# ruolin/strawberry

Measured on AMD Instinct MI355X. Metric: loci/s, EM-to-convergence (+ FPKM/TPM epilogue), C3, higher is better.
Workload: dtype f64; 1 GPU; C3 human-scale synthetic: 60000 loci/GPU, niso~1+Geom(0.25), nrow~LogNormal(ln30,1), 2e8 fragments; loci_per_gpu=60000, fragments_per_gpu=200000086, collective=none (one rank), steps_pipelined=True

## Files before the change

### include/sbgpu.h

```cpp
#ifndef SBGPU_H_
#define SBGPU_H_

#include <stdint.h>

#ifdef __cplusplus
extern "C" {
#endif

#define SBGPU_VERSION_MAJOR 0
#define SBGPU_VERSION_MINOR 1

#define SBGPU_OK 0
#define SBGPU_EINVAL (-1)
#define SBGPU_EHIP (-2)
#define SBGPU_ENODEV (-3)
#define SBGPU_ENOMEM (-4)
#define SBGPU_ESHAPE (-5)
#define SBGPU_EUNSUPPORTED (-6)
#define SBGPU_ERCCL (-7)

#define SBGPU_EM_OK 0
#define SBGPU_EM_INIT_EMPTY 1
#define SBGPU_EM_DENOM_ZERO 2
#define SBGPU_EM_MAXITER 3
// ... 11 lines not shown
   const int64_t *row_off;
   const int64_t *iso_off;
   const int64_t *f_off;
   const int32_t *count;
   const double *F;
} sbgpu_batch_t;

typedef struct {
   int32_t total_mapped_reads;
   int32_t effective_len_norm;
   int32_t filter_by_expression;
   int32_t reserved;
   double insert_mean;
   double min_isoform_frac;
} sbgpu_abundance_params_t;

const char *sbgpu_version(void);
const char *sbgpu_last_error(void);
const char *sbgpu_build_id(void);
int sbgpu_device_count(void);

int sbgpu_init(int device, sbgpu_ctx_t **ctx_out);
int sbgpu_finalize(sbgpu_ctx_t *ctx);
int64_t sbgpu_release_idle_memory(void);
int sbgpu_device_info(sbgpu_ctx_t *ctx, int64_t out[8]);
int sbgpu_synchronize(sbgpu_ctx_t *ctx, void *stream);

int sbgpu_plan_create(sbgpu_ctx_t *ctx, int64_t n_loci, const int64_t *row_off,
                      const int64_t *iso_off, const int64_t *f_off,
                      sbgpu_plan_t **plan_out);
int sbgpu_plan_destroy(sbgpu_plan_t *plan);
int sbgpu_plan_info(const sbgpu_plan_t *plan, int64_t out[8]);
int sbgpu_plan_classes(const sbgpu_plan_t *plan, int64_t *out, int cap);

int sbgpu_plan_locus_kinds(const sbgpu_plan_t *plan, int8_t *out);

int sbgpu_em_run_device(sbgpu_ctx_t *ctx, const sbgpu_plan_t *plan,
                        const int32_t *d_count, const double *d_F,
                        double *d_theta, int32_t *d_status, int32_t *d_iters,
                        void *stream);

int sbgpu_em_run_device_split(sbgpu_ctx_t *ctx, const sbgpu_plan_t *plan, const int32_t *d_count, const double *d_F,
                              double *d_theta, int32_t *d_status, int32_t *d_iters, void *fork_stream,
                              void *join_stream);

int sbgpu_em_run_device_f32(sbgpu_ctx_t *ctx, const sbgpu_plan_t *plan,
                            const int32_t *d_count, const float *d_F,
                            float *d_theta, int32_t *d_status, int32_t *d_iters,
                            void *stream);

int sbgpu_em_run_device_bias(sbgpu_ctx_t *ctx, const sbgpu_plan_t *plan, const int32_t *d_count, const double *d_F,
                             const double *d_row_bias, const double *d_iso_bias, double *d_theta, int32_t *d_status,
                             int32_t *d_iters, void *stream);
int sbgpu_em_run_device_bias_f32(sbgpu_ctx_t *ctx, const sbgpu_plan_t *plan, const int32_t *d_count, const float *d_F,
                                 const float *d_row_bias, const float *d_iso_bias, float *d_theta, int32_t *d_status,
                                 int32_t *d_iters, void *stream);

int sbgpu_set_timing(sbgpu_ctx_t *ctx, int on);
int sbgpu_last_stage_ms(sbgpu_ctx_t *ctx, int cap, float *ms, const char **names);

int sbgpu_em_last_kernel_ms(sbgpu_ctx_t *ctx, float ms[6]);

int sbgpu_em_last_phase_ms(sbgpu_ctx_t *ctx, float *ms, int cap);

int sbgpu_em_batch(sbgpu_ctx_t *ctx, const sbgpu_batch_t *host_batch,
                   double *theta_out, int32_t *status_out, int32_t *iters_out);
// ... 406 lines not shown
```

### strawberry_amd/_lib.py

```python
import ctypes as C
import os

HERE = os.path.dirname(os.path.abspath(__file__))
LIB_PATH = os.environ.get("SBGPU_LIB") or os.path.join(HERE, "lib", "libsbgpu.so")

SBGPU_OK = 0
SBGPU_EINVAL = -1
SBGPU_ESHAPE = -5
SBGPU_EUNSUPPORTED = -6
SBGPU_ERCCL = -7
EM_UNSOLVED = -1
EM_OK, EM_INIT_EMPTY, EM_DENOM_ZERO, EM_MAXITER = 0, 1, 2, 3
STATUS_NAMES = {0: "OK", 1: "INIT_EMPTY", 2: "DENOM_ZERO", 3: "MAXITER"}

SYMBOLS = [
    "sbgpu_version", "sbgpu_build_id", "sbgpu_last_error", "sbgpu_device_count", "sbgpu_init", "sbgpu_finalize",
    "sbgpu_device_info", "sbgpu_synchronize", "sbgpu_plan_create", "sbgpu_plan_destroy", "sbgpu_plan_info",
    "sbgpu_plan_classes", "sbgpu_plan_locus_kinds", "sbgpu_em_run_device", "sbgpu_em_run_device_f32", "sbgpu_em_run_device_bias", "sbgpu_em_run_device_bias_f32", "sbgpu_em_last_kernel_ms",
    "sbgpu_set_timing", "sbgpu_em_last_phase_ms", "sbgpu_last_stage_ms", "sbgpu_pair_mates_host", "sbgpu_pair_mates_device", "sbgpu_matepairs_destroy", "sbgpu_matepairs_info",
    "sbgpu_matepairs_pairs", "sbgpu_matepairs_export", "sbgpu_assign_reads_host", "sbgpu_assign_reads_device",
    "sbgpu_bam_index_host", "sbgpu_bam_decode_host", "sbgpu_bam_decode_device", "sbgpu_bamreads_destroy", "sbgpu_bamreads_info",
    "sbgpu_bamreads_reads", "sbgpu_bamreads_export",
    "sbgpu_comm_unique_id", "sbgpu_comm_init", "sbgpu_comm_info", "sbgpu_comm_rccl_ranks", "sbgpu_comm_destroy",
    "sbgpu_allreduce_sum_f64", "sbgpu_allreduce_sum_i64", "sbgpu_allreduce_sum_f64_host", "sbgpu_allreduce_sum_i64_host",
    "sbgpu_insert_pdf_table", "sbgpu_binweight_device", "sbgpu_binweight_host",
    "sbgpu_exonbin_device", "sbgpu_exonbin_host", "sbgpu_segments_host", "sbgpu_hit_features", "sbgpu_frag_lens_host",
    "sbgpu_bins_create", "sbgpu_bins_create_device", "sbgpu_bins_destroy", "sbgpu_quantify_host", "sbgpu_quantify_device",
    "sbgpu_annotation_pin", "sbgpu_annotation_unpin", "sbgpu_annotation_unpin_matching", "sbgpu_release_idle_memory",
    "sbgpu_bins_export_weights", "sbgpu_collapse_pairs_host", "sbgpu_uniq_destroy", "sbgpu_uniq_info", "sbgpu_uniq_export",
    "sbgpu_collapse_pairs_device", "sbgpu_uniq_dev_destroy", "sbgpu_uniq_dev_info", "sbgpu_uniq_dev_hits", "sbgpu_uniq_dev_export", "sbgpu_bins_info", "sbgpu_bins_grouping", "sbgpu_bins_export",
    "sbgpu_format_value", "sbgpu_format_gtf_transcript", "sbgpu_format_context_row", "sbgpu_format_context_row_seq",
    "sbgpu_binseq_device", "sbgpu_binseq_host", "sbgpu_em_batch", "sbgpu_abundance_device", "sbgpu_tpm_device",
    "sbgpu_quantify_resident", "sbgpu_allreduce_max_i64", "sbgpu_allreduce_max_i64_host", "sbgpu_comm_init_host",
    "sbgpu_front_stream_begin", "sbgpu_front_stream_push", "sbgpu_front_stream_end", "sbgpu_front_stream_info", "sbgpu_front_stream_hits",
    "sbgpu_front_stream_destroy", "sbgpu_em_run_device_split",
    "sbgpu_bgzf_index_host", "sbgpu_bgzf_inflate_host", "sbgpu_bgzf_inflate_device", "sbgpu_bam_index_device", "sbgpu_bam_index_device_info", "sbgpu_front_stream_push_bgzf",
    "sbgpu_context_table_host", "sbgpu_context_table_keep", "sbgpu_context_table_device",
    "sbgpu_bootstrap_counts_host", "sbgpu_bootstrap_counts_device", "sbgpu_em_bootstrap_device",
    "sbgpu_replicate_stats_host", "sbgpu_replicate_stats_device", "sbgpu_bootstrap_keep", "sbgpu_abundance_bootstrap_device",
    "sbgpu_locus_abundance_host", "sbgpu_locus_abundance_device", "sbgpu_locus_bootstrap_device",
    "sbgpu_fragment_assign_host", "sbgpu_fragment_assign_device",
]


class SbgpuError(RuntimeError):
    pass


class sbgpu_batch_t(C.Structure):
    _fields_ = [
        ("n_loci", C.c_int64),
        ("row_off", C.c_void_p),
        ("iso_off", C.c_void_p),
        ("f_off", C.c_void_p),
        ("count", C.c_void_p),
        ("F", C.c_void_p),
    ]


class sbgpu_abundance_params_t(C.Structure):
    _fields_ = [
        ("total_mapped_reads", C.c_int32),
        ("effective_len_norm", C.c_int32),
        ("filter_by_expression", C.c_int32),
        ("reserved", C.c_int32),
        ("insert_mean", C.c_double),
        ("min_isoform_frac", C.c_double),
    ]


class sbgpu_insert_t(C.Structure):
    _fields_ = [
        ("mean", C.c_double),
        ("sd", C.c_double),
# ... 100 lines not shown

def build():
    import subprocess
    subprocess.check_call(["make", "-s", "-C", os.path.join(HERE, "csrc")])


def load():
    global _lib
    if _lib is not None:
        return _lib
    if not os.path.exists(LIB_PATH):
        raise SbgpuError(
            "%s is missing: build it with `make -C strawberry_amd/csrc` (or __graft_entry__.build()). "
            "There is no CPU fallback." % LIB_PATH)
    try:
        import torch
    except ImportError:
        pass
    L = C.CDLL(LIB_PATH)
    vp, i64p = C.c_void_p, C.POINTER(C.c_int64)
    L.sbgpu_version.restype = C.c_char_p
    L.sbgpu_last_error.restype = C.c_char_p
    L.sbgpu_build_id.restype = C.c_char_p
    L.sbgpu_device_count.restype = C.c_int
    L.sbgpu_init.argtypes = [C.c_int, C.POINTER(vp)]
    L.sbgpu_finalize.argtypes = [vp]
    L.sbgpu_device_info.argtypes = [vp, i64p]
    L.sbgpu_synchronize.argtypes = [vp, vp]
    L.sbgpu_plan_create.argtypes = [vp, C.c_int64, vp, vp, vp, C.POINTER(vp)]
    L.sbgpu_plan_destroy.argtypes = [vp]
    L.sbgpu_plan_info.argtypes = [vp, i64p]
    L.sbgpu_plan_classes.argtypes = [vp, i64p, C.c_int]
    L.sbgpu_plan_locus_kinds.argtypes = [vp, vp]
    L.sbgpu_em_last_kernel_ms.argtypes = [vp, C.POINTER(C.c_float)]
    L.sbgpu_set_timing.argtypes = [vp, C.c_int]
    L.sbgpu_last_stage_ms.argtypes = [vp, C.c_int, C.POINTER(C.c_float), C.POINTER(C.c_char_p)]
    L.sbgpu_comm_unique_id.argtypes = [vp]
    L.sbgpu_comm_init.argtypes = [vp, C.c_int, C.c_int, vp, C.POINTER(vp)]
    L.sbgpu_comm_info.argtypes = [vp, C.POINTER(C.c_int), C.POINTER(C.c_int)]
    L.sbgpu_comm_rccl_ranks.argtypes = [vp, C.POINTER(C.c_int)]
    L.sbgpu_comm_destroy.argtypes = [vp]
    L.sbgpu_allreduce_sum_f64.argtypes = [vp, vp, C.c_int64, vp]
    L.sbgpu_allreduce_sum_i64.argtypes = [vp, vp, C.c_int64, vp]
    L.sbgpu_allreduce_sum_f64_host.argtypes = [vp, vp, C.c_int64]
    L.sbgpu_allreduce_sum_i64_host.argtypes = [vp, vp, C.c_int64]
    L.sbgpu_em_last_phase_ms.argtypes = [vp, C.POINTER(C.c_float), C.c_int]
    L.sbgpu_em_run_device.argtypes = [vp, vp, vp, vp, vp, vp, vp, vp]
    L.sbgpu_em_run_device_f32.argtypes = [vp, vp, vp, vp, vp, vp, vp, vp]
    L.sbgpu_em_run_device_split.argtypes = [vp, vp, vp, vp, vp, vp, vp, vp, vp]
    L.sbgpu_em_run_device_bias.argtypes = [vp] * 10
    L.sbgpu_em_run_device_bias_f32.argtypes = [vp] * 10
    L.sbgpu_em_batch.argtypes = [vp, C.POINTER(sbgpu_batch_t), vp, vp, vp]
    L.sbgpu_abundance_device.argtypes = [vp, vp, vp, vp, vp, C.POINTER(sbgpu_abundance_params_t), vp, vp, vp, vp, vp]
    L.sbgpu_tpm_device.argtypes = [vp, C.c_int64, vp, vp, vp, vp, vp]
    L.sbgpu_insert_pdf_table.argtypes = [C.POINTER(sbgpu_insert_t), C.c_int32, vp]
    L.sbgpu_binweight_device.argtypes = [vp, C.c_int64, vp, vp, vp, vp, vp, vp, C.c_int32, C.c_int32, C.c_int32,
                                         C.c_int32, vp, vp]
    L.sbgpu_exonbin_device.argtypes = [vp, C.POINTER(sbgpu_annotation_t), C.POINTER(sbgpu_hits_t), C.c_int32, C.c_int32,
                                       vp, vp, vp]
    L.sbgpu_exonbin_host.argtypes = [vp, C.POINTER(sbgpu_annotation_t), C.POINTER(sbgpu_hits_t), C.c_int32, C.c_int32,
                                     vp, vp]
    L.sbgpu_segments_host.argtypes = [C.c_int64, vp, vp, vp, vp, vp, vp, vp, C.c_int64]
    L.sbgpu_segments_host.restype = C.c_int64
    L.sbgpu_frag_lens_host.argtypes = [C.POINTER(sbgpu_annotation_t), C.POINTER(sbgpu_hits_t), C.c_int32, vp, vp]
    L.sbgpu_frag_lens_host.restype = C.c_int64
    L.sbgpu_hit_features.argtypes = [C.c_int, vp, vp, vp, C.c_int, vp, vp, vp, vp, vp, vp]
# ... 111 lines not shown
```

### strawberry_amd/csrc/em_device.h

```cpp
#pragma once

#include <hip/hip_runtime.h>
#include <stdint.h>

#include <type_traits>

#include "device_common.h"

namespace sb {

constexpr int kMaxIter = 1000;
constexpr double kThetaLimit = 1e-2;
constexpr double kThetaLimitSq = 0x1.a36e2eb1c432bp-14;
constexpr double kRowEps = 1e-5;

constexpr int kMaxCPLv = 8;
constexpr int32_t kStOk = 0, kStInitEmpty = 1, kStDenomZero = 2, kStMaxIter = 3;
constexpr int32_t kStRunning = 4;

template <class T>
struct EmArgsT {
   const int64_t *row_off;
   const int64_t *iso_off;
   const int64_t *f_off;
   const int32_t *count;
   const T *F;
   T *theta;
   int32_t *status;
   int32_t *iters;
   const T *row_bias = nullptr;
   const T *iso_bias = nullptr;
};
typedef EmArgsT<double> EmArgs;

struct ClassDesc {
   int32_t block_begin;
   int32_t n;
   int32_t loci_off;
   int32_t shape;
};
// ... 955 lines not shown
{
   __shared__ T s_red[NWAVES > 0 ? 2 * (kMaxCPLv + 1) * 8 * NWAVES : 1];
   set_flush_denormals<T>();
   if (NWAVES > 0) __builtin_amdgcn_s_setprio(3);
#ifdef SB_STAMPS
   const unsigned long long st0 = sb_now();
#endif
   const int n_batches = ph.total_blocks ? *ph.total_blocks : ph.n_batches;
   for (int b = (int)blockIdx.x; b < n_batches; b += (int)gridDim.x) {
   if (NWAVES > 0 && b != (int)blockIdx.x) __syncthreads();
   const int c = find_class(ph.table, ph.n_classes, b);
   const ClassDesc d = ph.table[c];
#ifdef SB_STAMPS
   if ((threadIdx.x & 63) == 0 && NWAVES == 0) {
      const unsigned wg = (blockIdx.x * (blockDim.x >> 6) + (threadIdx.x >> 6)) & (kStampWaves - 1);
      sb_debug_stamps[wg * 8 + 0] = st0;
      sb_debug_stamps[wg * 8 + 1] = sb_now();
      const unsigned hw = __builtin_amdgcn_s_getreg((31 << 11) | 4), xcc = __builtin_amdgcn_s_getreg((3 << 11) | 20);
      sb_debug_stamps[wg * 8 + 6] = ((xcc & 7u) << 10) | (((hw >> 8) & 0xFFu) << 2) | ((hw >> 4) & 3u);
   }
#endif
   ClassArgs cls;
   cls.loci = ph.lists_in + d.loci_off;
   cls.n = ph.n_in[c];
   cls.out = ph.lists_out;
   cls.out_count = ph.n_out;
   cls.route = ph.route;
   cls.next_table = ph.next_table;
   cls.it_limit = ph.it_limit;
   cls.resume = ph.resume;
   cls.batch = b - d.block_begin;
   const int layout = d.shape & 0xFF;
   const int lbG = (d.shape >> 16) & 0xFF;
#define SB_BODY(CPLV, CLV, RHALF)                                                                  \
   case (CPLV - 1) + 8 * ilog2(CLV):                                                               \
      em_tile_body<T, CPLV, CLV, tile_rows(CPLV, RHALF, RH), NWAVES>(a, cls, lbG, s_red);          \
      break;
   switch (layout) {
      SB_BODY(1, 1, 8)
      SB_BODY(2, 1, 4)
      SB_BODY(3, 1, 4)
      SB_BODY(4, 1, 4)
      SB_BODY(5, 1, 3)
      SB_BODY(6, 1, 3)
      SB_BODY(7, 1, 2)
      SB_BODY(8, 1, 2)
      SB_BODY(5, 2, 3)
      SB_BODY(6, 2, 3)
      SB_BODY(7, 2, 2)
      SB_BODY(8, 2, 2)
      SB_BODY(5, 4, 3)
      SB_BODY(6, 4, 3)
      SB_BODY(7, 4, 2)
      SB_BODY(8, 4, 2)
      SB_BODY(5, 8, 3)
      SB_BODY(6, 8, 3)
      SB_BODY(7, 8, 2)
      SB_BODY(8, 8, 2)
   default: break;
   }
#undef SB_BODY
   }
}

#ifndef SB_LAT_MAXTILE
#define SB_LAT_MAXTILE 32
#endif
constexpr int kLatMaxTile = SB_LAT_MAXTILE;
constexpr int lat_shape(int cpl, int lb_cl, int r) { return (cpl - 1) | (lb_cl << 2) | (r << 8); }
#ifndef SB_LAT_OCC
#define SB_LAT_OCC 2
#endif
#ifdef SB_COMPILE_LAT_KERNEL
__global__ __launch_bounds__(64, SB_LAT_OCC) void em_lat_kernel(EmArgs a, PhaseArgs ph)
{
   set_fp64_flush_denormals();
   const int n_batches = ph.total_blocks ? *ph.total_blocks : ph.n_batches;
   for (int b = (int)blockIdx.x; b < n_batches; b += (int)gridDim.x) {
      const int c = find_class(ph.table, ph.n_classes, b);
      const ClassDesc d = ph.table[c];
      ClassArgs cls;
      cls.loci = ph.lists_in + d.loci_off;
      cls.n = ph.n_in[c];
      cls.out = ph.lists_out;
      cls.out_count = ph.n_out;
      cls.route = ph.route;
      cls.next_table = ph.next_table;
      cls.it_limit = ph.it_limit;
      cls.resume = ph.resume;
      cls.batch = b - d.block_begin;
#define SB_LAT(CPLV, CLV, RV)                                                             \
   case lat_shape(CPLV, ilog2(CLV), RV):                                                  \
      if constexpr (CPLV * RV <= kLatMaxTile)                                             \
         em_tile_body<double, CPLV, CLV, RV, 0, true>(a, cls, 6, nullptr);                \
// ... 298 lines not shown
```

### strawberry_amd/csrc/plan.cpp

```cpp
#include "plan.h"

#include <algorithm>
#include <atomic>
#include <cstdlib>
#include <thread>
#include <map>
#include <tuple>

#include "../../include/sbgpu.h"

namespace sb {

static int64_t predicted_iterations(int64_t nrow, int64_t niso)
{
   if (nrow <= 0 || niso <= 0) return 0;
   const double r = (double)nrow / (double)niso;
   const double w = r < 0.5 ? 0.10 : r < 0.75 ? 0.60 : r < 1.25 ? 1.00 : r < 1.5 ? 0.80 : r < 2 ? 0.55 : r < 3 ? 0.35 : r < 5 ? 0.27
                  : r < 10 ? 0.20 : 0.17;
   const double it = 80.0 * w * (double)((niso < 24 ? niso : 24) + 18);
   return (int64_t)(it < 1000.0 ? it : 1000.0);
}


static int pow2ceil(int64_t x)
{
   int p = 1;
   while (p < x) p <<= 1;
   return p;
}
static unsigned plan_threads(int64_t n_items)
{
   unsigned nt = std::thread::hardware_concurrency();
   if (nt > 16) nt = 16;
   if (const char *e = std::getenv("SBGPU_HOST_THREADS")) nt = (unsigned)std::atoi(e);
   if (nt < 1) nt = 1;
   if (nt > 64) nt = 64;
   if ((int64_t)nt * 8192 > n_items) nt = (unsigned)std::max<int64_t>(1, n_items / 8192);
   return nt;
}
template <class F>
static void parallel_ranges(int64_t n, unsigned nt, F f)
{
   if (nt <= 1) {
      f((int64_t)0, n, 0u);
      return;
   }
   std::vector<std::thread> pool;
   for (unsigned t = 0; t < nt; ++t) pool.emplace_back([=]() { f(n * t / nt, n * (t + 1) / nt, t); });
   for (auto &th : pool) th.join();
}

static int ilog2i(int x)
{
   int l = 0;
   while ((1 << l) < x) ++l;
   return l;
}

static double lat_cycles(int cpl, int lb_cl, int r, int lb_gr)
{
   const double row_reduce = lb_gr == 0 ? 0.0 : lb_gr == 1 ? 32.0 : 18.0 * (lb_gr - 2) + 19.0;
   return 6.0 * cpl + 12.0 * r * cpl + 18.0 * r * lb_cl + 62.0 * r + cpl * row_reduce + 18.0 * cpl + 21.0 * lb_cl + 60.0;
}

bool lat_layout_for(int64_t nrow, int64_t niso, double lambda, LatLayout *out)
{
   bool found = false;
   double best = 0.0;
   for (int lb_cl = 0; lb_cl <= 4; ++lb_cl) {
      const int cl = 1 << lb_cl;
      const int64_t cpl = (niso + cl - 1) / cl;
      if (cpl > 4 || cpl < 1) continue;
      if (lb_cl > 0 && (niso + cl / 2 - 1) / (cl / 2) <= 1) continue;
      for (int r : kLatRows) {
         if (r * cpl > kLatMaxTileElems) continue;
         const int gr = 64 / cl;
         if ((std::max<int64_t>(nrow, 1) + r - 1) / r > gr) continue;
         const int lb_gr = ilog2i(gr);
         const double cyc = lat_cycles((int)cpl, lb_cl, r, lb_gr);
         const double score = cyc * (1.0 + lambda * (double)(gr * cl) / 64.0);
         if (!found || score < best) {
            found = true;
            best = score;
            out->cpl = (int)cpl, out->lb_cl = lb_cl, out->r = r, out->lbG = lb_gr + lb_cl, out->cycles = cyc;
         }
      }
   }
   return found;
}
// ... 58 lines not shown
         p.algorithmic_bytes += bytes_t[t];
         bad |= bad_t[t];
      }
      if (bad & 1) {
         *err = "plan: malformed locus (need niso >= 1, nrow >= 0, f_off step == nrow*niso)";
         return SBGPU_EINVAL;
      }
      if (bad & 2) {
         *err = "plan: a locus has more than 512 isoforms";
         return SBGPU_ESHAPE;
      }
   }
   const int64_t simd_lanes = (int64_t)n_cu * 4 * 64;
   int wave_rmult = tune.wave_rmult;
   if (wave_rmult != 1 && wave_rmult != 2 && wave_rmult != 4) {
      wave_rmult = (wave_lanes_base <= 16 * simd_lanes) ? 2 : 4;
   }

   std::vector<int> limits = tune.phase_limits;
   std::vector<double> lambdas = tune.phase_lambda;
   if (limits.empty() && tune.phases_auto && n_loci >= 4096) {
      limits = {32, 128, 512};
      lambdas = {8.0, 2.0, 0.25};
   }
   {
      std::vector<int> ok;
      for (int v : limits)
         if (v > (ok.empty() ? 1 : ok.back()) && v < SBGPU_EM_MAX_ITER && ok.size() < 6) ok.push_back(v);
      limits = ok;
      while (lambdas.size() < limits.size()) lambdas.push_back(lambdas.empty() ? 1.0 : lambdas.back());
   }
   const bool phased = !limits.empty();

   typedef std::tuple<int, int, int, int> ClassKey;
   struct Local {
      std::map<ClassKey, int> slot_of;
      std::vector<SizeClass> found;
      int64_t n_stream = 0;
   };
   std::vector<Local> local(nt);
   std::vector<int64_t> work_of((size_t)n_loci);
   parallel_ranges(n_loci, nt, [&](int64_t lb, int64_t le, unsigned t) {
      Local &L = local[t];
      int last_slot = -1;
      ClassKey last_key(-1, -1, -1, -1);
      for (int64_t l = lb; l < le; ++l) {
         const int64_t nrow = row_off[l + 1] - row_off[l];
         const int64_t niso = iso_off[l + 1] - iso_off[l];
         work_of[(size_t)l] = tune.order_by_work ? nrow * niso : predicted_iterations(nrow, niso) * ((int64_t)1 << 32) + nrow * niso;
         int kind = kStream, layout = 0, CPL = 0, CL = 0, rmult = 1, R = 0, G = 0, lbG = 0;
         if (niso <= kMaxTileC) {
            layout_for(niso, &CPL, &CL);
            layout = layout_id(CPL, CL);
            bool placed = false;
            {
               const int Rw = tile_rows(CPL, wave_rmult);
               const int64_t lanes = (int64_t)pow2ceil(std::max<int64_t>(1, (nrow + Rw - 1) / Rw)) * CL;
               LatLayout ll;
               if (lanes <= 64 && (!phased || lat_layout_for(nrow, niso, 0.0, &ll))) {
                  kind = (wave_rmult == 1) ? kWaveH : (wave_rmult == 2 ? kWave1 : kWave2);
                  rmult = wave_rmult;
                  R = Rw;
                  G = (int)lanes;
                  lbG = ilog2i(G);
                  placed = true;
               }
            }
            for (int tall = tune.light_block ? 0 : 1; tall < 2 && !placed; ++tall) {
               const int rm = tall ? kBlockTallRh : kBlockRh;
               if ((int64_t)(kBlockThreads / CL) * tile_rows(CPL, rm) >= nrow) {
                  kind = tall ? kBlockTall : kBlock;
                  rmult = rm;
                  R = tile_rows(CPL, rm);
                  G = kBlockThreads;
                  lbG = 6;
                  placed = true;
               }
            }
         }
         if (kind == kStream) {
            layout = CPL = CL = R = G = lbG = 0;
            rmult = 1;
            ++L.n_stream;
         }
         const ClassKey key(kind, layout, rmult, G);
         int slot;
         if (key == last_key) {
            slot = last_slot;
         } else {
            auto it = L.slot_of.find(key);
            if (it == L.slot_of.end()) {
               it = L.slot_of.emplace(key, (int)L.found.size()).first;
               SizeClass k;
               k.kind = kind, k.layout = layout, k.CPL = CPL, k.CL = CL, k.rmult = rmult, k.R = R, k.G = G, k.lbG = lbG;
               L.found.push_back(std::move(k));
            }
            slot = it->second;
            last_key = key;
            last_slot = slot;
         }
         SizeClass &sc = L.found[(size_t)slot];
         sc.loci.push_back((int32_t)l);
         sc.work += (kind == kStream) ? nrow * niso : (int64_t)(G / std::max(1, CL)) * R * CPL * CL;
      }
   });
   std::map<ClassKey, SizeClass> merged;
   for (unsigned t = 0; t < nt; ++t) {
      p.n_stream_loci += local[t].n_stream;
      for (auto &kv : local[t].slot_of) {
         SizeClass &src = local[t].found[(size_t)kv.second];
         auto it = merged.find(kv.first);
         if (it == merged.end()) {
            merged.emplace(kv.first, std::move(src));
         } else {
            it->second.loci.insert(it->second.loci.end(), src.loci.begin(), src.loci.end());
            it->second.work += src.work;
         }
      }
   }
   std::vector<std::pair<ClassKey, SizeClass>> by_key;
   for (auto &kv : merged) by_key.emplace_back(kv.first, std::move(kv.second));
   p.n_rows = row_off[n_loci];
   p.n_iso = iso_off[n_loci];
   p.n_elem = f_off[n_loci];

   const int64_t max_waves = tune.max_waves > 0 ? tune.max_waves : (int64_t)1 << 20;
   int64_t waves_wanted = 0;
   {
      std::atomic<size_t> next(0);
      auto sorter = [&]() {
         for (;;) {
            const size_t ci = next.fetch_add(1);
            if (ci >= by_key.size()) break;
            std::vector<int32_t> &loci = by_key[ci].second.loci;
            std::sort(loci.begin(), loci.end(), [&](int32_t x, int32_t y) {
               const int64_t wx = work_of[(size_t)x], wy = work_of[(size_t)y];
// ... 45 lines not shown
         if (sc.kind == kWaveH || sc.kind == kWave1 || sc.kind == kWave2) wave_loci.insert(wave_loci.end(), sc.loci.begin(), sc.loci.end());
      if (!wave_loci.empty()) {
         p.first_limit = limits[0];
         p.lat.resize(limits.size());
         for (size_t ph = 0; ph < limits.size(); ++ph) {
            LatPhase &lp = p.lat[ph];
            lp.it_limit = ph + 1 < limits.size() ? limits[ph + 1] : SBGPU_EM_MAX_ITER;
            lp.route.assign((size_t)n_loci, -1);
            const double lambda = lambdas[ph];
            if (lambda < 0.0) {
               lp.repack = true;
               for (const SizeClass &sc : p.classes) {
                  if (!(sc.kind == kWaveH || sc.kind == kWave1 || sc.kind == kWave2)) continue;
                  SizeClass c2 = sc;
                  c2.loci.clear();
                  for (int32_t l : sc.loci) lp.route[(size_t)l] = (int32_t)lp.classes.size();
                  lp.capacity.push_back((int32_t)sc.loci.size());
                  lp.max_blocks += sc.n_blocks;
                  lp.classes.push_back(std::move(c2));
               }
               continue;
            }
            std::vector<LatLayout> lay(wave_loci.size());
            parallel_ranges((int64_t)wave_loci.size(), nt, [&](int64_t b, int64_t e, unsigned) {
               for (int64_t k = b; k < e; ++k) {
                  const int32_t l = wave_loci[(size_t)k];
                  lat_layout_for(row_off[l + 1] - row_off[l], iso_off[l + 1] - iso_off[l], lambda, &lay[(size_t)k]);
               }
            });
            std::map<ClassKey, int> slot;
            std::vector<double> cyc;
            for (size_t k = 0; k < wave_loci.size(); ++k) {
               const LatLayout &ll = lay[k];
               const ClassKey key(ll.cpl, ll.lb_cl, ll.r, ll.lbG);
               auto it = slot.find(key);
               if (it == slot.end()) {
                  it = slot.emplace(key, (int)lp.classes.size()).first;
                  SizeClass sc;
                  sc.kind = kLat;
                  sc.CPL = ll.cpl, sc.CL = 1 << ll.lb_cl, sc.R = ll.r, sc.rmult = ll.r;
                  sc.layout = (ll.cpl - 1) | (ll.lb_cl << 2);
                  sc.lbG = ll.lbG, sc.G = 1 << ll.lbG;
                  sc.block_threads = 64;
                  lp.classes.push_back(sc);
                  lp.capacity.push_back(0);
                  cyc.push_back(ll.cycles);
               }
               lp.capacity[(size_t)it->second] += 1;
               lp.route[(size_t)wave_loci[k]] = it->second;
            }
            std::vector<int> order(lp.classes.size()), where(lp.classes.size());
            for (size_t i = 0; i < order.size(); ++i) order[i] = (int)i;
            std::stable_sort(order.begin(), order.end(), [&](int x, int y) { return cyc[(size_t)x] > cyc[(size_t)y]; });
            std::vector<SizeClass> cls2;
            std::vector<int32_t> cap2;
            for (size_t i = 0; i < order.size(); ++i) {
               where[(size_t)order[i]] = (int)i;
               cls2.push_back(lp.classes[(size_t)order[i]]);
               cap2.push_back(lp.capacity[(size_t)order[i]]);
            }
            lp.classes.swap(cls2);
            lp.capacity.swap(cap2);
            for (int32_t l : wave_loci) lp.route[(size_t)l] = where[(size_t)lp.route[(size_t)l]];
            lp.max_blocks = 0;
            for (size_t i = 0; i < lp.classes.size(); ++i) {
               const int lpw = 64 >> lp.classes[i].lbG;
               lp.max_blocks += (lp.capacity[i] + lpw - 1) / lpw;
// ... 9 lines not shown
```

### strawberry_amd/csrc/plan.h

```cpp
#pragma once

#include <cstdint>
#include <vector>

namespace sb {

enum ClassKind : int { kWaveH = 0, kWave1, kWave2, kBlock, kBlockTall, kStream, kNumKinds };
constexpr int kLat = kNumKinds;
constexpr int kBlockThreads = 256;
constexpr int kBlockRh = 2;
constexpr int kBlockTallRh = 12;

struct SizeClass {
   int kind = kWave1;
   int layout = 0;
   int CPL = 0, CL = 0;
   int rmult = 2;
   int R = 0;
   int G = 0;
   int lbG = 0;
   std::vector<int32_t> loci;
   int n_blocks = 0;
   int block_threads = 0;
   int64_t work = 0;
   int64_t pred = 0;
};

struct LatPhase {
   bool repack = false;
   int it_limit = 0;
   std::vector<SizeClass> classes;
   std::vector<int32_t> capacity;
   std::vector<int32_t> route;
   int64_t max_blocks = 0;
};

struct HostPlan {
   int64_t n_loci = 0, n_rows = 0, n_iso = 0, n_elem = 0;
   int64_t algorithmic_bytes = 0;
   int64_t n_stream_loci = 0;
   std::vector<SizeClass> classes;
   int first_limit = 1000;
   double grid_scale = 1.0;
   std::vector<LatPhase> lat;
};

constexpr int kLayoutRHalf[8] = {8, 4, 4, 4, 3, 3, 2, 2};
inline int tile_rows(int cpl, int rh)
{
   const int r = kLayoutRHalf[cpl - 1] * rh;
   return (r * cpl > 128) ? 128 / cpl : r;
}
inline int layout_id(int cpl, int cl)
{
   int lb = 0;
   while ((1 << lb) < cl) ++lb;
   return (cpl - 1) + 8 * lb;
}
inline void layout_for(int64_t niso, int *cpl, int *cl)
{
   int c = 1;
   while (niso > 8 * c) c *= 2;
   *cl = c;
   *cpl = (int)((niso + c - 1) / c);
}
constexpr int kMaxTileC = 64;
constexpr int kMaxStreamIso = 512;

struct PlanTuning {
   int wave_rmult = 0;
   bool light_block = true;
   int64_t max_waves = 0;
   bool classes_by_prediction = true;
   bool order_by_work = false;
   bool phases_auto = false;
   std::vector<int> phase_limits;
   std::vector<double> phase_lambda;
};

constexpr int kLatRows[6] = {1, 2, 3, 4, 6, 8};
constexpr int kLatMaxTileElems = 32;
struct LatLayout {
   int cpl = 0, lb_cl = 0, r = 0, lbG = 0;
   double cycles = 0.0;
};
bool lat_layout_for(int64_t nrow, int64_t niso, double lambda, LatLayout *out);

int build_host_plan(int64_t n_loci, const int64_t *row_off, const int64_t *iso_off,
                    const int64_t *f_off, int n_cu, const PlanTuning &tune, HostPlan *out,
                    const char **err);

}
```

### strawberry_amd/csrc/sbgpu_api.hip

```cpp
#include <hip/hip_runtime.h>

#include <cstdio>
#include <cstdlib>
#include <chrono>
#include <cmath>
#include <cstring>
#include <mutex>
#include <new>
#include <string>
#include <system_error>
#include <thread>
#include <vector>

#include "../../include/sbgpu.h"
#include "api_internal.h"
#include "binweight_device.h"
#include "em_device.h"
#include "em_wide.h"
#include "plan.h"

namespace {

thread_local std::string g_err;

// ... 623 lines not shown

int sbgpu_synchronize(sbgpu_ctx_t *c, void *stream)
{
   if (!c) return fail(SBGPU_EINVAL, "sbgpu_synchronize: null ctx");
   HIP_TRY(hipStreamSynchronize((hipStream_t)stream));
   if (c->wide_error && *c->wide_error) {
      *c->wide_error = 0;
      return fail(SBGPU_EHIP, "a barrier of the wide-locus EM kernel timed out: the loci it served have no result");
   }
   return SBGPU_OK;
}

int sbgpu_plan_destroy(sbgpu_plan_t *p)
{
   if (!p) return SBGPU_OK;
   if (p->ctx) (void)hipSetDevice(p->ctx->device);
   sb::dev_give(p->d_arena, p->arena_cap);
   if (p->graph_exec) (void)hipGraphExecDestroy(p->graph_exec);
   delete p;
   return SBGPU_OK;
}

int sbgpu_plan_create(sbgpu_ctx_t *c, int64_t n_loci, const int64_t *row_off, const int64_t *iso_off,
                      const int64_t *f_off, sbgpu_plan_t **plan_out)
{
   if (!c || !plan_out) return fail(SBGPU_EINVAL, "sbgpu_plan_create: null argument");
   *plan_out = nullptr;
   sbgpu_plan *p = new (std::nothrow) sbgpu_plan();
   if (!p) return fail(SBGPU_ENOMEM, "sbgpu_plan_create: out of host memory");
   p->ctx = c;
   const char *err = "";
   sb::PlanTuning tune;
   if (const char *e = sb::exp_env("SBGPU_WAVE_RMULT")) tune.wave_rmult = std::atoi(e);
   if (const char *e = sb::exp_env("SBGPU_MAX_WAVES")) tune.max_waves = std::atoll(e);
   if (const char *e = sb::exp_env("SBGPU_LIGHT_BLOCK")) tune.light_block = std::atoi(e) != 0;
   if (const char *e = sb::exp_env("SBGPU_ORDER")) tune.order_by_work = std::string(e) == "work";
   if (const char *e = sb::exp_env("SBGPU_CLASS_ORDER")) tune.classes_by_prediction = std::string(e) != "cost";
   auto parse_list = [](const char *ev, auto conv, auto *out) {
      std::string spec = ev;
      size_t pos = 0;
      while (pos < spec.size()) {
         size_t q = spec.find(',', pos);
         if (q == std::string::npos) q = spec.size();
         out->push_back(conv(spec.substr(pos, q - pos)));
         pos = q + 1;
      }
   };
   if (const char *e = sb::exp_env("SBGPU_PHASES")) {
      tune.phases_auto = false;
      parse_list(e, [](const std::string &t) { return std::atoi(t.c_str()); }, &tune.phase_limits);
   }
   if (const char *e = sb::exp_env("SBGPU_PHASE_LAMBDA"))
      parse_list(e, [](const std::string &t) { return (!t.empty() && (t[0] == 't' || t[0] == 'T')) ? -1.0 : std::atof(t.c_str()); }, &tune.phase_lambda);
   const bool timing = std::getenv("SBGPU_HOST_TIMING") != nullptr;
   auto now = []() { return std::chrono::duration<double>(std::chrono::steady_clock::now().time_since_epoch()).count(); };
   double t_stage = now();
   auto stage = [&](const char *name) {
      if (timing) {
         const double t = now();
         std::fprintf(stderr, "sbgpu_plan_create: %-12s %.2f ms\n", name, (t - t_stage) * 1e3);
         t_stage = t;
      }
   };
   int rc = sb::build_host_plan(n_loci, row_off, iso_off, f_off, c->n_cu, tune, &p->host, &err);
   stage("size classes");
   if (rc != SBGPU_OK) {
// ... 125 lines not shown
      ld.d_route = (int32_t *)(p->d_arena + o_lroute[i]);
      ld.d_counts = (int32_t *)(p->d_arena + o_lcnt[i]);
      ld.d_total = (int32_t *)(p->d_arena + o_ltot[i]);
      ld.d_lists = (int32_t *)(p->d_arena + o_llist[i]);
      ld.n_classes = (int)lp.classes.size();
      ld.it_limit = lp.it_limit;
      ld.repack = lp.repack;
      ld.grid = (int)std::min<int64_t>(std::max<int64_t>(lp.max_blocks, 1), 32768);
   }
   p->d_row_keep = (uint8_t *)(p->d_arena + o_keep);
   p->d_locus_sum = (double *)(p->d_arena + o_sum);
   p->d_epi_ticket = (unsigned *)(p->d_arena + o_tick);
   p->d_wide_table = (sb::WideDesc *)(p->d_arena + o_wtab);
   p->d_wide_bufs = (double *)(p->d_arena + o_wbuf);
   std::vector<char> stage_buf(staged, 0);
   if (n_loci > 0) {
      std::memcpy(stage_buf.data() + o_row, row_off, nb);
      std::memcpy(stage_buf.data() + o_iso, iso_off, nb);
      std::memcpy(stage_buf.data() + o_f, f_off, nb);
   }
   int32_t *h_loci = (int32_t *)(stage_buf.data() + o_loci);
   sb::ClassDesc *table = (sb::ClassDesc *)(stage_buf.data() + o_tab);
   int32_t *h_cn = (int32_t *)(stage_buf.data() + o_cn);
   if (!wide_table.empty()) std::memcpy(stage_buf.data() + o_wtab, wide_table.data(), wide_table.size() * sizeof(sb::WideDesc));
   for (size_t i = 0; i < nlat; ++i) {
      const sb::LatPhase &lp = p->host.lat[i];
      sb::ClassDesc *lt = (sb::ClassDesc *)(stage_buf.data() + o_ltab[i]);
      int32_t loff = 0;
      for (size_t ci = 0; ci < lp.classes.size(); ++ci) {
         const sb::SizeClass &sc = lp.classes[ci];
         lt[ci].block_begin = 0;
         lt[ci].n = lp.capacity[ci];
         lt[ci].loci_off = loff;
         lt[ci].shape = sc.layout | (sc.rmult << 8) | (sc.lbG << 16);
         loff += lp.capacity[ci];
      }
      std::memcpy(stage_buf.data() + o_lroute[i], lp.route.data(), lp.route.size() * sizeof(int32_t));
   }
   size_t off = 0;
   size_t max_stream_iso = 0;
   for (int k = 0; k < sb::kNumKinds; ++k) p->launches[k] = KindLaunch();
   for (size_t ci = 0; ci < ncls; ++ci) {
      const sb::SizeClass &sc = p->host.classes[ci];
      KindLaunch &kl = p->launches[sc.kind];
      if (kl.n_classes == 0) {
         kl.first_class = (int)ci;
         kl.d_table = p->d_tables + ci;
         kl.block_threads = sc.block_threads;
      }
      table[ci].block_begin = kl.n_blocks;
      table[ci].n = (int32_t)sc.loci.size();
      table[ci].loci_off = (int32_t)off;
      table[ci].shape = sc.layout | (sc.rmult << 8) | (sc.lbG << 16);
      h_cn[ci] = table[ci].n;
      kl.n_blocks += sc.n_blocks;
      kl.n_classes += 1;
      std::memcpy(h_loci + off, sc.loci.data(), sc.loci.size() * sizeof(int32_t));
      p->loci_off.push_back((int64_t)off);
      off += sc.loci.size();
      if (sc.kind == sb::kStream) {
         for (int32_t l : sc.loci) {
            size_t k = (size_t)(iso_off[l + 1] - iso_off[l]);
            if (k > max_stream_iso) max_stream_iso = k;
         }
      }
   }
   stage("staging");
   if ((e = hipMemcpy(p->d_arena, stage_buf.data(), staged, hipMemcpyHostToDevice)) != hipSuccess) return bail(e, "hipMemcpy(plan)");
   if (wide_buf_doubles && (e = hipMemset(p->d_wide_bufs, 0, wide_buf_doubles * sizeof(double))) != hipSuccess) return bail(e, "hipMemset(plan)");
   stage("upload");
   size_t npad = 1;
   while (npad < max_stream_iso && npad < 64) npad <<= 1;
   if (max_stream_iso > 64) npad = 64 * ((max_stream_iso + 63) / 64);
   p->stream_lds_bytes = (3 + sb::kStreamThreads / 64) * npad * sizeof(double);
   *plan_out = p;
   return SBGPU_OK;
}

int sbgpu_plan_info(const sbgpu_plan_t *p, int64_t out[8])
{
   if (!p || !out) return fail(SBGPU_EINVAL, "sbgpu_plan_info: null argument");
   out[0] = p->host.n_loci;
   out[1] = p->host.n_rows;
   out[2] = p->host.n_iso;
   out[3] = p->host.n_elem;
   out[4] = (int64_t)p->host.classes.size();
// ... 331 lines not shown
      HIP_TRY(hipEventElapsedTime(&ms[k], c->t0[k], c->t1[k]));
   }
   return SBGPU_OK;
}

#ifdef SB_STAMPS
int sbgpu_debug_touch_streams(sbgpu_ctx_t *c, double *d_buf)
{
   for (int i = 0; i < kAuxStreams; ++i) {
      hipLaunchKernelGGL(sum_kernel, dim3(i + 1), dim3(1024), 0, c->aux[i], (int64_t)0, d_buf, d_buf + 1);
      HIP_TRY(hipGetLastError());
   }
   hipLaunchKernelGGL(sum_kernel, dim3(20), dim3(1024), 0, c->stream, (int64_t)0, d_buf, d_buf + 1);
   hipLaunchKernelGGL(sum_kernel, dim3(30), dim3(1024), 0, (hipStream_t)0, (int64_t)0, d_buf, d_buf + 1);
   HIP_TRY(hipDeviceSynchronize());
   return SBGPU_OK;
}

int sbgpu_debug_read_stamps(void *out, size_t bytes)
{
   HIP_TRY(hipDeviceSynchronize());
   std::vector<unsigned long long> part(bytes / 8), all(bytes / 8, 0ull);
   hipError_t (*readers[])(void *, size_t) = {sb::read_stamps_wave_h, sb::read_stamps_wave_1, sb::read_stamps_wave_2,
                                              sb::read_stamps_block, sb::read_stamps_block_tall};
   for (auto rd : readers) {
      HIP_TRY(rd(part.data(), part.size() * 8));
      for (size_t i = 0; i < all.size(); ++i) all[i] = std::max(all[i], part[i]);
   }
   std::memcpy(out, all.data(), all.size() * 8);
   return SBGPU_OK;
}
#endif

int sbgpu_plan_locus_kinds(const sbgpu_plan_t *p, int8_t *out)
{
   if (!p || (!out && p->host.n_loci)) return fail(SBGPU_EINVAL, "sbgpu_plan_locus_kinds: null argument");
   for (const sb::SizeClass &sc : p->host.classes)
      for (int32_t l : sc.loci) out[l] = (int8_t)sc.kind;
   return SBGPU_OK;
}

int sbgpu_em_batch(sbgpu_ctx_t *c, const sbgpu_batch_t *b, double *theta_out, int32_t *status_out,
                   int32_t *iters_out)
{
   if (!c || !b) return fail(SBGPU_EINVAL, "sbgpu_em_batch: null argument");
   if (b->n_loci == 0) return SBGPU_OK;
   if (!theta_out || !status_out) return fail(SBGPU_EINVAL, "sbgpu_em_batch: null output");
   if (b->n_loci < 0 || !b->row_off || !b->iso_off || !b->f_off) return fail(SBGPU_EINVAL, "sbgpu_em_batch: bad n_loci or null offset array");
   const int64_t n_rows = b->row_off[b->n_loci], n_iso = b->iso_off[b->n_loci], n_el = b->f_off[b->n_loci];
   if (n_rows < 0 || n_iso < 0 || n_el < 0 || (n_rows && !b->count) || (n_el && !b->F))
      return fail(SBGPU_EINVAL, "sbgpu_em_batch: negative size or null count / F array");
   sbgpu_plan_t *p = nullptr;
   int32_t *d_count = nullptr, *d_status = nullptr, *d_iters = nullptr;
   double *d_F = nullptr, *d_theta = nullptr;
   auto cleanup = [&]() {
      (void)hipFree(d_count);
      (void)hipFree(d_status);
      (void)hipFree(d_iters);
      (void)hipFree(d_F);
      (void)hipFree(d_theta);
      sbgpu_plan_destroy(p);
   };
#define TRY_CLEAN(expr)                                                                       \
   do {                                                                                       \
      hipError_t e_ = (expr);                                                                 \
      if (e_ != hipSuccess) {                                                                 \
// ... 312 lines not shown
```

### strawberry_amd/em.py

```python
import ctypes as C

import numpy as np

from . import _lib
from ._lib import EM_DENOM_ZERO, EM_INIT_EMPTY, EM_MAXITER, EM_OK, SbgpuError


def _torch():
    import torch
    if not torch.cuda.is_available():
        raise SbgpuError("no HIP device visible: the EM hot path has no CPU fallback")
    return torch


class Context:

    def __init__(self, device=0):
        self.L = _lib.load()
        h = C.c_void_p()
        _lib.check(self.L.sbgpu_init(int(device), C.byref(h)), "sbgpu_init")
        self.h = h
        self.device = int(device)

    def device_info(self):
# ... 11 lines not shown
            self.close()
        except Exception:
            pass


_default_ctx = {}


def default_context(device=0):
    if device not in _default_ctx:
        _default_ctx[device] = Context(device)
    return _default_ctx[device]


class Plan:

    def __init__(self, ctx, row_off, iso_off, f_off):
        self.ctx = ctx
        self.row_off = np.ascontiguousarray(row_off, np.int64)
        self.iso_off = np.ascontiguousarray(iso_off, np.int64)
        self.f_off = np.ascontiguousarray(f_off, np.int64)
        n = len(self.row_off) - 1
        if len(self.iso_off) != n + 1 or len(self.f_off) != n + 1:
            raise ValueError("offset arrays must all have n_loci+1 entries")
        h = C.c_void_p()
        _lib.check(ctx.L.sbgpu_plan_create(ctx.h, n, self.row_off.ctypes.data, self.iso_off.ctypes.data,
                                           self.f_off.ctypes.data, C.byref(h)), "sbgpu_plan_create")
        self.h = h
        self.n_loci = n

    def info(self):
        out = (C.c_int64 * 8)()
        _lib.check(self.ctx.L.sbgpu_plan_info(self.h, out), "sbgpu_plan_info")
        return {"n_loci": out[0], "n_rows": out[1], "n_iso": out[2], "n_elem": out[3], "n_classes": out[4],
                "n_stream_loci": out[5], "algorithmic_bytes": out[6], "n_wide_loci": out[7]}

    def classes(self):
        cap = 1024
        out = (C.c_int64 * (6 * cap))()
        n = self.ctx.L.sbgpu_plan_classes(self.h, out, cap)
        keys = ("kind", "C", "R", "G", "n_loci", "n_waves")
        return [dict(zip(keys, out[i * 6:(i + 1) * 6])) for i in range(min(n, cap))]

    def locus_kinds(self):
        out = np.zeros(max(self.n_loci, 1), np.int8)
        _lib.check(self.ctx.L.sbgpu_plan_locus_kinds(self.h, out.ctypes.data), "sbgpu_plan_locus_kinds")
        return out[:self.n_loci]

    def close(self):
        if self.h:
            self.ctx.L.sbgpu_plan_destroy(self.h)
            self.h = None

    def __del__(self):
        try:
            self.close()
        except Exception:
            pass


class EmBatchSolver:

    def __init__(self, batch, ctx=None, device=0, d_F=None):
        torch = _torch()
        self.torch = torch
        self.ctx = ctx or default_context(device)
        self.dev = torch.device("cuda", self.ctx.device)
        self.batch = batch
        self.plan = Plan(self.ctx, batch.row_off, batch.iso_off, batch.f_off)
        n, n_iso = batch.n_loci, int(batch.iso_off[-1])
        self.d_count = torch.from_numpy(np.ascontiguousarray(batch.count, np.int32)).to(self.dev)
        self.d_F = d_F if d_F is not None else torch.from_numpy(np.ascontiguousarray(batch.F, np.float64)).to(self.dev)
        self.d_length = torch.from_numpy(np.ascontiguousarray(batch.length, np.int32)).to(self.dev)
        self.d_theta = torch.zeros(max(n_iso, 1), dtype=torch.float64, device=self.dev)
        self.d_status = torch.full((max(n, 1),), -1, dtype=torch.int32, device=self.dev)
# ... 191 lines not shown
```

Measured before the change: 87.25 million loci/s.

## Bin wave loci into height-specialized tile classes instead of full-height tiles

Adds a table of shorter tile heights per wave layout. The planner now picks the smallest height that covers each locus's rows and keys size classes on that height. The kernel dispatches on layout plus height, so short loci no longer pad to full tile height, which wastes lanes and iterations. In exchange there are more size classes, more kernel template instantiations, and possibly more launches or blocks. An env var restores full-height tiles.

```diff
diff --git a/include/sbgpu.h b/include/sbgpu.h
--- a/include/sbgpu.h
+++ b/include/sbgpu.h
@@ -67,6 +67,10 @@
 int sbgpu_plan_destroy(sbgpu_plan_t *plan);
 int sbgpu_plan_info(const sbgpu_plan_t *plan, int64_t out[8]);
 int sbgpu_plan_classes(const sbgpu_plan_t *plan, int64_t *out, int cap);
+int sbgpu_plan_class_heights(const sbgpu_plan_t *plan, int64_t *out, int cap);
+int sbgpu_plan_loci_host(int64_t n_loci, const int64_t *row_off, const int64_t *iso_off, const int64_t *f_off,
+                         int n_cu, int full_height, int64_t *out);
+int sbgpu_tile_heights(int kind, int cpl, int cl, int32_t *out);
 
 int sbgpu_plan_locus_kinds(const sbgpu_plan_t *plan, int8_t *out);
 
diff --git a/strawberry_amd/_lib.py b/strawberry_amd/_lib.py
--- a/strawberry_amd/_lib.py
+++ b/strawberry_amd/_lib.py
@@ -40,6 +40,7 @@
     "sbgpu_replicate_stats_host", "sbgpu_replicate_stats_device", "sbgpu_bootstrap_keep", "sbgpu_abundance_bootstrap_device",
     "sbgpu_locus_abundance_host", "sbgpu_locus_abundance_device", "sbgpu_locus_bootstrap_device",
     "sbgpu_fragment_assign_host", "sbgpu_fragment_assign_device",
+    "sbgpu_plan_class_heights", "sbgpu_plan_loci_host", "sbgpu_tile_heights",
 ]
 
 
@@ -206,6 +207,9 @@
     L.sbgpu_plan_info.argtypes = [vp, i64p]
     L.sbgpu_plan_classes.argtypes = [vp, i64p, C.c_int]
     L.sbgpu_plan_locus_kinds.argtypes = [vp, vp]
+    L.sbgpu_plan_class_heights.argtypes = [vp, i64p, C.c_int]
+    L.sbgpu_plan_loci_host.argtypes = [C.c_int64, vp, vp, vp, C.c_int, C.c_int, vp]
+    L.sbgpu_tile_heights.argtypes = [C.c_int, C.c_int, C.c_int, vp]
     L.sbgpu_em_last_kernel_ms.argtypes = [vp, C.POINTER(C.c_float)]
     L.sbgpu_set_timing.argtypes = [vp, C.c_int]
     L.sbgpu_last_stage_ms.argtypes = [vp, C.c_int, C.POINTER(C.c_float), C.POINTER(C.c_char_p)]
diff --git a/strawberry_amd/csrc/em_device.h b/strawberry_amd/csrc/em_device.h
--- a/strawberry_amd/csrc/em_device.h
+++ b/strawberry_amd/csrc/em_device.h
@@ -6,6 +6,7 @@
 #include <type_traits>
 
 #include "device_common.h"
+#include "plan.h"
 
 namespace sb {
 
@@ -1027,6 +1028,17 @@
    cls.batch = b - d.block_begin;
    const int layout = d.shape & 0xFF;
    const int lbG = (d.shape >> 16) & 0xFF;
+   if constexpr (RH == kHeightsRh && NWAVES == 0) {
+#define SB_TILE(CPLV, CLV, HV)                                                                      \
+   case tile_key((CPLV - 1) + 8 * ilog2(CLV), HV):                                                  \
+      em_tile_body<T, CPLV, CLV, HV, NWAVES>(a, cls, lbG, s_red);                                   \
+      break;
+      switch (tile_key(layout, (d.shape >> 24) & 0xFF)) {
+         SB_WAVE_TILES(SB_TILE)
+      default: break;
+      }
+#undef SB_TILE
+   } else {
 #define SB_BODY(CPLV, CLV, RHALF)                                                                  \
    case (CPLV - 1) + 8 * ilog2(CLV):                                                               \
       em_tile_body<T, CPLV, CLV, tile_rows(CPLV, RHALF, RH), NWAVES>(a, cls, lbG, s_red);          \
@@ -1055,6 +1067,7 @@
    default: break;
    }
 #undef SB_BODY
+   }
    }
 }
 
diff --git a/strawberry_amd/csrc/plan.cpp b/strawberry_amd/csrc/plan.cpp
--- a/strawberry_amd/csrc/plan.cpp
+++ b/strawberry_amd/csrc/plan.cpp
@@ -55,6 +55,19 @@
    int l = 0;
    while ((1 << l) < x) ++l;
    return l;
+}
+
+int tile_heights(int kind, int cpl, int cl, bool full_only, int *out)
+{
+   const int rh = kind == kWaveH ? 1 : kind == kWave1 ? 2 : kind == kWave2 ? 4 : kind == kBlock ? kBlockRh : kBlockTallRh;
+   int n = 0;
+   if (!full_only && kind == kWave1) {
+      for (int i = 0; i < kNumWaveTiles; ++i)
+         if (kWaveTiles[i].cpl == cpl && kWaveTiles[i].cl == cl) out[n++] = kWaveTiles[i].h;
+      if (n > 0) return n;
+   }
+   out[n++] = tile_rows(cpl, rh);
+   return n;
 }
 
 static double lat_cycles(int cpl, int lb_cl, int r, int lb_gr)
@@ -179,7 +192,7 @@
    }
    const bool phased = !limits.empty();
 
-   typedef std::tuple<int, int, int, int> ClassKey;
+   typedef std::tuple<int, int, int, int, int> ClassKey;
    struct Local {
       std::map<ClassKey, int> slot_of;
       std::vector<SizeClass> found;
@@ -190,12 +203,12 @@
    parallel_ranges(n_loci, nt, [&](int64_t lb, int64_t le, unsigned t) {
       Local &L = local[t];
       int last_slot = -1;
-      ClassKey last_key(-1, -1, -1, -1);
+      ClassKey last_key(-1, -1, -1, -1, -1);
       for (int64_t l = lb; l < le; ++l) {
          const int64_t nrow = row_off[l + 1] - row_off[l];
          const int64_t niso = iso_off[l + 1] - iso_off[l];
          work_of[(size_t)l] = tune.order_by_work ? nrow * niso : predicted_iterations(nrow, niso) * ((int64_t)1 << 32) + nrow * niso;
-         int kind = kStream, layout = 0, CPL = 0, CL = 0, rmult = 1, R = 0, G = 0, lbG = 0;
+         int kind = kStream, layout = 0, CPL = 0, CL = 0, rmult = 1, R = 0, G = 0, lbG = 0, H = 0;
          if (niso <= kMaxTileC) {
             layout_for(niso, &CPL, &CL);
             layout = layout_id(CPL, CL);
@@ -229,8 +242,15 @@
             layout = CPL = CL = R = G = lbG = 0;
             rmult = 1;
             ++L.n_stream;
-         }
-         const ClassKey key(kind, layout, rmult, G);
+         } else {
+            const int GR = G / CL;
+            const int64_t need = std::max<int64_t>(1, (nrow + GR - 1) / GR);
+            int hs[kMaxHeights];
+            const int nh = tile_heights(kind, CPL, CL, !tune.heights, hs);
+            H = hs[nh - 1];
+            for (int k = nh - 1; k >= 0 && hs[k] >= need; --k) H = hs[k];
+         }
+         const ClassKey key(kind, layout, rmult, G, H);
          int slot;
          if (key == last_key) {
             slot = last_slot;
@@ -239,7 +259,7 @@
             if (it == L.slot_of.end()) {
                it = L.slot_of.emplace(key, (int)L.found.size()).first;
                SizeClass k;
-               k.kind = kind, k.layout = layout, k.CPL = CPL, k.CL = CL, k.rmult = rmult, k.R = R, k.G = G, k.lbG = lbG;
+               k.kind = kind, k.layout = layout, k.CPL = CPL, k.CL = CL, k.rmult = rmult, k.R = R, k.H = H, k.G = G, k.lbG = lbG;
                L.found.push_back(std::move(k));
             }
             slot = it->second;
@@ -248,7 +268,7 @@
          }
          SizeClass &sc = L.found[(size_t)slot];
          sc.loci.push_back((int32_t)l);
-         sc.work += (kind == kStream) ? nrow * niso : (int64_t)(G / std::max(1, CL)) * R * CPL * CL;
+         sc.work += (kind == kStream) ? nrow * niso : (int64_t)(G / std::max(1, CL)) * H * CPL * CL;
       }
    });
    std::map<ClassKey, SizeClass> merged;
@@ -360,7 +380,7 @@
             std::vector<double> cyc;
             for (size_t k = 0; k < wave_loci.size(); ++k) {
                const LatLayout &ll = lay[k];
-               const ClassKey key(ll.cpl, ll.lb_cl, ll.r, ll.lbG);
+               const ClassKey key(ll.cpl, ll.lb_cl, ll.r, ll.lbG, 0);
                auto it = slot.find(key);
                if (it == slot.end()) {
                   it = slot.emplace(key, (int)lp.classes.size()).first;
diff --git a/strawberry_amd/csrc/plan.h b/strawberry_amd/csrc/plan.h
--- a/strawberry_amd/csrc/plan.h
+++ b/strawberry_amd/csrc/plan.h
@@ -17,6 +17,7 @@
    int CPL = 0, CL = 0;
    int rmult = 2;
    int R = 0;
+   int H = 0;
    int G = 0;
    int lbG = 0;
    std::vector<int32_t> loci;
@@ -64,12 +65,52 @@
    *cl = c;
    *cpl = (int)((niso + c - 1) / c);
 }
+#define SB_WAVE_TILES(X)                                                                        \
+   X(1, 1, 16)                                                                                  \
+   X(2, 1, 5) X(2, 1, 6) X(2, 1, 8) X(3, 1, 5) X(3, 1, 6) X(3, 1, 8) X(4, 1, 5) X(4, 1, 6) X(4, 1, 8) \
+   X(5, 1, 4) X(5, 1, 5) X(5, 1, 6) X(6, 1, 4) X(6, 1, 5) X(6, 1, 6)                            \
+   X(7, 1, 3) X(7, 1, 4) X(8, 1, 3) X(8, 1, 4)                                                  \
+   X(5, 2, 4) X(5, 2, 6) X(6, 2, 4) X(6, 2, 6)                                                  \
+   X(7, 2, 3) X(7, 2, 4) X(8, 2, 3) X(8, 2, 4)                                                  \
+   X(5, 4, 4) X(5, 4, 6) X(6, 4, 4) X(6, 4, 6)                                                  \
+   X(7, 4, 4) X(8, 4, 4)                                                                        \
+   X(5, 8, 6) X(6, 8, 6) X(7, 8, 4) X(8, 8, 4)
+constexpr int kHeightsRh = 2;
+constexpr int tile_key(int layout, int h) { return layout | (h << 8); }
+constexpr int kMaxHeights = 8;
+int tile_heights(int kind, int cpl, int cl, bool full_only, int *out);
+struct TileEntry {
+   int cpl, cl, h;
+};
+#define SB_TILE_ENTRY(CPLV, CLV, HV) {CPLV, CLV, HV},
+constexpr TileEntry kWaveTiles[] = {SB_WAVE_TILES(SB_TILE_ENTRY)};
+#undef SB_TILE_ENTRY
+constexpr int kNumWaveTiles = (int)(sizeof(kWaveTiles) / sizeof(TileEntry));
+constexpr bool wave_tiles_well_formed()
+{
+   for (int cl = 1; cl <= 8; cl *= 2)
+      for (int cpl = 1; cpl <= 8; ++cpl) {
+         if (cl > 1 && cpl < 5) continue;
+         int n = 0, last = 0;
+         for (int i = 0; i < kNumWaveTiles; ++i)
+            if (kWaveTiles[i].cpl == cpl && kWaveTiles[i].cl == cl) {
+               if (kWaveTiles[i].h <= last) return false;
+               last = kWaveTiles[i].h;
+               ++n;
+            }
+         const int r = kLayoutRHalf[cpl - 1] * kHeightsRh;
+         if (n < 1 || n > kMaxHeights || last != ((r * cpl > 128) ? 128 / cpl : r)) return false;
+      }
+   return true;
+}
+static_assert(wave_tiles_well_formed(), "SB_WAVE_TILES: per layout rising, at most kMaxHeights, the last one the full height");
 constexpr int kMaxTileC = 64;
 constexpr int kMaxStreamIso = 512;
 
 struct PlanTuning {
    int wave_rmult = 0;
    bool light_block = true;
+   bool heights = true;
    int64_t max_waves = 0;
    bool classes_by_prediction = true;
    bool order_by_work = false;
diff --git a/strawberry_amd/csrc/sbgpu_api.hip b/strawberry_amd/csrc/sbgpu_api.hip
--- a/strawberry_amd/csrc/sbgpu_api.hip
+++ b/strawberry_amd/csrc/sbgpu_api.hip
@@ -679,6 +679,7 @@
    const char *err = "";
    sb::PlanTuning tune;
    if (const char *e = sb::exp_env("SBGPU_WAVE_RMULT")) tune.wave_rmult = std::atoi(e);
+   if (const char *e = sb::exp_env("SBGPU_FULL_HEIGHT")) tune.heights = std::atoi(e) == 0;
    if (const char *e = sb::exp_env("SBGPU_MAX_WAVES")) tune.max_waves = std::atoll(e);
    if (const char *e = sb::exp_env("SBGPU_LIGHT_BLOCK")) tune.light_block = std::atoi(e) != 0;
    if (const char *e = sb::exp_env("SBGPU_ORDER")) tune.order_by_work = std::string(e) == "work";
@@ -870,7 +871,7 @@
          lt[ci].block_begin = 0;
          lt[ci].n = lp.capacity[ci];
          lt[ci].loci_off = loff;
-         lt[ci].shape = sc.layout | (sc.rmult << 8) | (sc.lbG << 16);
+         lt[ci].shape = sc.layout | (sc.rmult << 8) | (sc.lbG << 16) | (sc.H << 24);
          loff += lp.capacity[ci];
       }
       std::memcpy(stage_buf.data() + o_lroute[i], lp.route.data(), lp.route.size() * sizeof(int32_t));
@@ -889,7 +890,7 @@
       table[ci].block_begin = kl.n_blocks;
       table[ci].n = (int32_t)sc.loci.size();
       table[ci].loci_off = (int32_t)off;
-      table[ci].shape = sc.layout | (sc.rmult << 8) | (sc.lbG << 16);
+      table[ci].shape = sc.layout | (sc.rmult << 8) | (sc.lbG << 16) | (sc.H << 24);
       h_cn[ci] = table[ci].n;
       kl.n_blocks += sc.n_blocks;
       kl.n_classes += 1;
@@ -1287,6 +1288,44 @@
 }
 #endif
 
+int sbgpu_plan_class_heights(const sbgpu_plan_t *p, int64_t *out, int cap)
+{
+   if (!p) return fail(SBGPU_EINVAL, "sbgpu_plan_class_heights: null plan");
+   const int n = (int)p->host.classes.size();
+   for (int i = 0; i < n && i < cap && out; ++i) out[i] = p->host.classes[(size_t)i].H;
+   return n;
+}
+
+int sbgpu_plan_loci_host(int64_t n_loci, const int64_t *row_off, const int64_t *iso_off, const int64_t *f_off,
+                         int n_cu, int full_height, int64_t *out)
+{
+   if (n_loci > 0 && !out) return fail(SBGPU_EINVAL, "sbgpu_plan_loci_host: null output");
+   sb::PlanTuning tune;
+   tune.heights = full_height == 0;
+   sb::HostPlan hp;
+   const char *err = "";
+   const int rc = sb::build_host_plan(n_loci, row_off, iso_off, f_off, n_cu, tune, &hp, &err);
+   if (rc != SBGPU_OK) return fail(rc, err);
+   for (size_t ci = 0; ci < hp.classes.size(); ++ci) {
+      const sb::SizeClass &sc = hp.classes[ci];
+      for (size_t k = 0; k < sc.loci.size(); ++k) {
+         int64_t *o = out + (int64_t)sc.loci[k] * 6;
+         o[0] = (int64_t)ci, o[1] = (int64_t)k, o[2] = sc.kind, o[3] = sc.layout, o[4] = sc.G, o[5] = sc.H;
+      }
+   }
+   return (int)hp.classes.size();
+}
+
+int sbgpu_tile_heights(int kind, int cpl, int cl, int32_t *out)
+{
+   if (!out || kind < 0 || kind >= sb::kStream || cpl < 1 || cpl > 8 || (cl != 1 && cl != 2 && cl != 4 && cl != 8))
+      return fail(SBGPU_EINVAL, "sbgpu_tile_heights: bad argument");
+   int hs[sb::kMaxHeights];
+   const int n = sb::tile_heights(kind, cpl, cl, false, hs);
+   for (int i = 0; i < n; ++i) out[i] = hs[i];
+   return n;
+}
+
 int sbgpu_plan_locus_kinds(const sbgpu_plan_t *p, int8_t *out)
 {
    if (!p || (!out && p->host.n_loci)) return fail(SBGPU_EINVAL, "sbgpu_plan_locus_kinds: null argument");
diff --git a/strawberry_amd/em.py b/strawberry_amd/em.py
--- a/strawberry_amd/em.py
+++ b/strawberry_amd/em.py
@@ -67,15 +67,27 @@
     def info(self):
         out = (C.c_int64 * 8)()
         _lib.check(self.ctx.L.sbgpu_plan_info(self.h, out), "sbgpu_plan_info")
+        per_height = {}
+        for c in self.classes():
+            if c["H"] > 0:
+                per_height[c["H"]] = per_height.get(c["H"], 0) + 1
         return {"n_loci": out[0], "n_rows": out[1], "n_iso": out[2], "n_elem": out[3], "n_classes": out[4],
-                "n_stream_loci": out[5], "algorithmic_bytes": out[6], "n_wide_loci": out[7]}
+                "n_stream_loci": out[5], "algorithmic_bytes": out[6], "n_wide_loci": out[7],
+                "classes_per_height": dict(sorted(per_height.items()))}
 
     def classes(self):
         cap = 1024
         out = (C.c_int64 * (6 * cap))()
         n = self.ctx.L.sbgpu_plan_classes(self.h, out, cap)
         keys = ("kind", "C", "R", "G", "n_loci", "n_waves")
-        return [dict(zip(keys, out[i * 6:(i + 1) * 6])) for i in range(min(n, cap))]
+        res = [dict(zip(keys, out[i * 6:(i + 1) * 6])) for i in range(min(n, cap))]
+        hs = (C.c_int64 * cap)()
+        if self.ctx.L.sbgpu_plan_class_heights(self.h, hs, cap) != n or n > cap:
+            raise RuntimeError("sbgpu_plan_class_heights: %d classes, sbgpu_plan_classes %d (room for %d)" % (
+                self.ctx.L.sbgpu_plan_class_heights(self.h, hs, cap), n, cap))
+        for i, c in enumerate(res):
+            c["H"] = hs[i]
+        return res
 
     def locus_kinds(self):
         out = np.zeros(max(self.n_loci, 1), np.int8)
```

New measurement: 87.40 million loci/s, median of 2. Within noise of the previous version (+0.2%).
